# ARISE-Initiative/robosuite

Hardware: NVIDIA H100
Metric: env-steps/sec (device-timed) Panda-Lift OSC_POSE @4096 envs per GPU (higher is better)
Workload: dtype f32

## Files before the change

robosuite_b200/csrc/b2s_capi.cu:

```cuda
#include "../../include/b2s.h"
#include "b2s_unit.cuh"
#include "b2s_snapshot.cuh"

#include <cmath>
#include <cstdio>
#include <cstdlib>
#include <cstring>
#include <map>
#include <algorithm>
#include <string>
#include <type_traits>
#include <vector>

static thread_local std::string g_err;
static int fail(int code, const std::string& msg) { g_err = msg; return code; }
#define CUDA_TRY(x) do { cudaError_t e_ = (x); if (e_ != cudaSuccess) return fail(B2S_ERR_CUDA, std::string(#x) + ": " + cudaGetErrorString(e_)); } while (0)

struct BlobRec { char name[48]; int32_t dtype, ndim, shape[4]; int64_t off, nbytes; };
struct Blob {
  const char* p; size_t n;
  const BlobRec* find(const char* name) const {
    int64_t cnt; memcpy(&cnt, p + 8, 8);
    const BlobRec* r = (const BlobRec*)(p + 16);
    for (int64_t i = 0; i < cnt; i++) if (!strcmp(r[i].name, name)) return r + i;
    return nullptr;
  }
  bool has(const char* name) const { return find(name) != nullptr; }
  uint64_t hash() const;
  const double* f64(const char* name, int64_t* count = nullptr) const {
    const BlobRec* r = find(name);
    if (!r || r->dtype != 0) throw std::string("model blob: missing f64 field ") + name;
    if (count) *count = r->nbytes / 8;
    return (const double*)(p + r->off);
  }
  const int* i32(const char* name, int64_t* count = nullptr) const {
    const BlobRec* r = find(name);
    if (!r || r->dtype != 1) throw std::string("model blob: missing i32 field ") + name;
    if (count) *count = r->nbytes / 4;
    return (const int*)(p + r->off);
  }
  int scalar_i(const char* name) const { return i32(name)[0]; }
  double scalar_f(const char* name) const { return f64(name)[0]; }
};
static const uint64_t FNV_BASIS = 1469598103934665603ull;
static uint64_t fnv1a(uint64_t h, const void* p, size_t n) {
  const unsigned char* c = (const unsigned char*)p;
  for (size_t i = 0; i < n; i++) { h ^= c[i]; h *= 1099511628211ull; }
  return h;
}
uint64_t Blob::hash() const {
  int64_t cnt; memcpy(&cnt, p + 8, 8);
  const BlobRec* r = (const BlobRec*)(p + 16);
  uint64_t h = FNV_BASIS;
  for (int64_t i = 0; i < cnt; i++) {
    const char* nm = r[i].name;
    if (!strcmp(nm, "opt_maxcon") || !strcmp(nm, "opt_maxefc") || !strcmp(nm, "opt_maxcon_small") || !strcmp(nm, "opt_maxefc_small")) continue;
    h = fnv1a(h, nm, strnlen(nm, sizeof(r[i].name)) + 1);
    h = fnv1a(h, &r[i].dtype, sizeof(int32_t) * 6);
    h = fnv1a(h, p + r[i].off, (size_t)r[i].nbytes);
  }
  return h;
}

struct ArrayInfo { void* ptr; int dtype; int ndim; int64_t shape[4]; };
struct SnapSecHost { std::string name; int64_t off, count; int dtype; void* ptr; };
#define SNAP_MAXSEC 128

struct b2s_sim {
  int n_env = 0, device = 0, precision = B2S_F32;
  int num_sms = 1;
  cudaStream_t stream = 0;
  std::vector<void*> allocs;
  std::map<std::string, ArrayInfo> arrays;
  WSLayout lay[B2S_NLAY]{};
  int slot = -1;
  int mc_small = 0, me_small = 0;
  int osc_in_tail = 0;
  int wpb0 = 8, wpb5s = 8, wpb5l = 4;
  size_t smem0 = 0, smem5s = 0, smem5l = 0;
  DModel<float> mf{};
  DModel<double> md{};
  DState<float> sf{};
  DState<double> sd{};
  CtrlCfgDev ctrl{};
  int has_ctrl = 0;
  int wpb_fused = 4;
  size_t smem_fused = 0;
  int64_t launches = 0;
  int nq = 0, nv = 0, nu = 0, nbody = 0, ngeom = 0, nsite = 0, maxcon = 0, maxefc = 0, ncg = 0, hc_stride = 0;
  std::vector<double> qpos0;
  std::vector<int> site_bodyid, cgid;
  std::map<std::string, std::vector<std::string>> names;
  int has_obs = 0, export_env_step = 1, dirty = 1, mode = 0, ngroups = 8;
  int ctrl_split = 1;
  std::vector<cudaStream_t> gstreams;
  std::vector<cudaEvent_t> gevents;
  cudaEvent_t in_event = nullptr;
  void* action_buf = nullptr;
  std::map<long long, cudaGraphExec_t> graphs;
  PhaseIO pio[B2S_NPIO];
  std::map<std::string, Region> reg;
  int* uq_ring = nullptr; int* uq_ovf = nullptr; int* uq_ctr = nullptr; int uq_cap = 0;
  int uq_wpb = 0, uq_stride = 0, uq_stride_large = 0, uq_wpb_large = 0, uq_nlarge = 0, uq_grid = 0;
  size_t uq_smem = 0;
#ifdef B2S_INSTR
  unsigned long long* uq_prof = nullptr;
#endif
  std::vector<double> xpos0_h, xquat0_h;
  std::vector<int> body_weldid_h;
  std::vector<int> geom_type_h;
  std::vector<double> geom_size_h, geom_friction_h, geom_rbound_h, geom_aabb_h, body_mass_h, body_inertia_h, dof_iw_h, body_iw_h;
  std::vector<double> geom_solref_h, geom_solimp_h, dof_damping_h, dof_armature_h, dof_frictionloss_h;
  double meaninertia_h = 1;
  int sc_words = 0;
  PerturbEntry* pert_ent = nullptr;
  PerturbItem* pert_item = nullptr;
  int pert_nitems = 0;
  int layout_version = 0, snap_version = -1;
  std::vector<SnapSecHost> snap;
  size_t snap_row_bytes = 0;
  uint64_t snap_sig = 0, blob_hash = 0;
  SnapSec* snap_dev = nullptr;
  std::vector<int> obs_tab_h, task_tab_h;
};

template <typename F> static auto with_real(b2s_sim* s, F&& f) { return s->precision == B2S_F32 ? f(s->mf, s->sf) : f(s->md, s->sd); }
template <typename M> struct RealOf;
template <typename R> struct RealOf<DModel<R>> { using type = R; };
template <typename M> using real_of = typename RealOf<std::remove_cv_t<std::remove_reference_t<M>>>::type;
static size_t real_size(const b2s_sim* s) { return s->precision == B2S_F32 ? sizeof(float) : sizeof(double); }

static int launch_set_const(b2s_sim* s, const uint8_t* mask);

template <typename T> static T* dev_upload(b2s_sim* s, const std::vector<T>& h) {
  T* d = nullptr;
  size_t n = h.size() ? h.size() : 1;
  if (cudaMalloc(&d, n * sizeof(T)) != cudaSuccess) throw std::string("cudaMalloc failed");
  s->allocs.push_back(d);
  if (h.size()) cudaMemcpy(d, h.data(), h.size() * sizeof(T), cudaMemcpyHostToDevice);
  cudaStreamSynchronize(cudaStreamLegacy);
  return d;
}
template <typename R> static const R* up_f(b2s_sim* s, const Blob& b, const char* name) {
  int64_t n; const double* p = b.f64(name, &n);
  std::vector<R> h(n);
  for (int64_t i = 0; i < n; i++) h[i] = (R)p[i];
  return dev_upload(s, h);
}
static const int* up_i(b2s_sim* s, const Blob& b, const char* name) {
  int64_t n; const int* p = b.i32(name, &n);
  std::vector<int> h(p, p + n);
  return dev_upload(s, h);
}
template <typename R> static const R* up_vec(b2s_sim* s, const std::vector<double>& v) {
  std::vector<R> h(v.size());
  for (size_t i = 0; i < v.size(); i++) h[i] = (R)v[i];
  return dev_upload(s, h);
}

static void h_quat2mat(double* M, const double* q) {
  double w = q[0], x = q[1], y = q[2], z = q[3];
  M[0] = w * w + x * x - y * y - z * z; M[1] = 2 * (x * y - w * z); M[2] = 2 * (x * z + w * y);
// ... 325 lines not shown
  if (osc_in_tail && sc < 672) sc = 672;
  L.scratch_size = sc; L.scratch = B.take(sc);
  L.hdr = B.take(8);
  L.total = B.o;
}

static void layout_row(const Dims& d, WSLayout& L) {
  LayB B;
  int nv = d.nv, nb = d.nb, ncg = d.ncg, ns = d.ns;
  L = WSLayout{};
  L.xpos = B.take(3 * nb); L.xquat = B.take(4 * nb); L.cdof = B.take(6 * nv); L.cvel = B.take(6 * nb);
  L.M = B.take(nv * nv); L.bias = B.take(nv); L.passive = B.take(nv); L.spos = B.take(3 * ns); L.smat = B.take(9 * ns);
  L.gpos = B.take(3 * ncg); L.gmat = B.take(9 * ncg);
  L.hdr = B.take(8);
  L.total = B.o;
}

static void make_io(const Dims& d, const WSLayout& S, const WSLayout& ROW, std::initializer_list<const char*> names, Region* out, int& n, int* words) {
  int nv = d.nv, nb = d.nb, ncg = d.ncg, ns = d.ns;
  auto a4 = [](int x) { return (x + 3) & ~3; };
  std::vector<Region> v;
  for (const char* nm : names) {
    std::string k = nm;
    Region r{0, 0, 0, 0};
#define REG(name, field, len_) if (k == name) { r.off = S.field; r.goff = ROW.field; r.len = a4(len_); }
    REG("xpos", xpos, 3 * nb) REG("xquat", xquat, 4 * nb) REG("cdof", cdof, 6 * nv) REG("cvel", cvel, 6 * nb) REG("M", M, nv * nv)
    REG("bias", bias, nv) REG("passive", passive, nv) REG("spos", spos, 3 * ns) REG("smat", smat, 9 * ns)
    REG("gpos", gpos, 3 * ncg) REG("gmat", gmat, 9 * ncg)
#undef REG
    if (r.len > 0) v.push_back(r);
  }
  std::sort(v.begin(), v.end(), [](const Region& a, const Region& b) { return a.goff < b.goff; });
  n = 0;
  if (words) *words = 0;
  for (const Region& r : v) {
    if (n > 0 && out[n - 1].off + out[n - 1].len == r.off && out[n - 1].goff + out[n - 1].len == r.goff) out[n - 1].len += r.len;
    else { if (n >= B2S_MAXREG) throw std::string("too many workspace spans"); out[n++] = r; }
  }
  if (words) for (int k = 0; k < n; k++) *words += out[k].len;
}

static void build_layouts(b2s_sim* s, int ncg, int hc_stride) {
  Dims d{s->nq, s->nv, s->nu, s->nbody, ncg, s->nsite, hc_stride};
  layout_full(d, s->maxcon, s->maxefc, s->lay[LAY_FULL]);
  layout_p0(d, s->lay[LAY_P0]);
  layout_tail(d, s->mc_small, s->me_small, s->osc_in_tail != 0, s->lay[LAY_TS]);
  layout_tail(d, s->maxcon, s->maxefc, s->osc_in_tail != 0, s->lay[LAY_TL]);
  layout_row(d, s->lay[LAY_ROW]);
  for (int k = 0; k < B2S_NPIO; k++) s->pio[k] = PhaseIO{};
  const WSLayout& ROW = s->lay[LAY_ROW];
  make_io(d, s->lay[LAY_P0], ROW, {"xpos", "xquat", "cdof", "cvel", "M", "bias", "passive", "spos", "smat", "gpos", "gmat"},
          s->pio[PIO_P0].store, s->pio[PIO_P0].nstore, nullptr);
  for (int t = 0; t < 2; t++) {
    const WSLayout& T = s->lay[t ? LAY_TL : LAY_TS];
    PhaseIO& early = s->pio[t ? PIO_TL : PIO_TS];
    PhaseIO& late = s->pio[t ? PIO_TL_LATE : PIO_TS_LATE];
    if (s->osc_in_tail) make_io(d, T, ROW, {"cdof", "cvel", "M", "bias", "passive", "xpos", "xquat", "spos", "smat"}, early.load, early.nload, &early.load_words);
    else {
      make_io(d, T, ROW, {"cdof", "M", "bias", "passive"}, early.load, early.nload, &early.load_words);
      make_io(d, T, ROW, {"xpos", "xquat", "spos", "smat"}, late.load, late.nload, &late.load_words);
    }
  }
}

template <typename F> static cudaError_t optin_max_smem(F fn, int device, int* limit_out = nullptr) {
  cudaFuncAttributes a;
  cudaError_t e = cudaFuncGetAttributes(&a, fn);
  if (e != cudaSuccess) return e;
  int optin = 0;
  e = cudaDeviceGetAttribute(&optin, cudaDevAttrMaxSharedMemoryPerBlockOptin, device);
  if (e != cudaSuccess) return e;
  int lim = optin - (int)a.sharedSizeBytes;
  if (limit_out) *limit_out = lim;
  return cudaFuncSetAttribute(fn, cudaFuncAttributeMaxDynamicSharedMemorySize, lim);
}

static int fit_wpb(size_t per_warp, int cap) {
  int w = cap;
  while (w > 1 && per_warp * w > 226 * 1024) w--;
  return w;
}
static int choose_blocks(b2s_sim* s) {
  size_t rsz = real_size(s);
  size_t pw0 = s->lay[LAY_P0].total * rsz, pws = s->lay[LAY_TS].total * rsz, pwl = s->lay[LAY_TL].total * rsz, pwf = s->lay[LAY_FULL].fused_stride * rsz;
  if (std::max(std::max(pw0, pws), std::max(pwl, pwf)) > 226 * 1024) return fail(B2S_ERR_UNSUPPORTED, "model workspace exceeds shared memory");
  auto pick = [&](size_t pw, int lb_threads, int lb_blocks) {
    int cap = lb_threads / 32, w = cap;
    while (w > 1 && (pw * w + 1024) * lb_blocks > 228 * 1024) w--;
    if ((pw * w + 1024) * lb_blocks > 228 * 1024) w = fit_wpb(pw, cap);
    return w;
  };
  s->wpb0 = pick(pw0, P0_THREADS, P0_BLOCKS);
  s->wpb5s = pick(pws, TAIL_THREADS, TAIL_BLOCKS);
  s->wpb5l = fit_wpb(pwl, TAIL_THREADS / 32);
  s->smem0 = pw0 * s->wpb0; s->smem5s = pws * s->wpb5s; s->smem5l = pwl * s->wpb5l;
  int wf = fit_wpb(pwf, 16);
  s->wpb_fused = wf; s->smem_fused = pwf * wf;
  if (getenv("B2S_VERBOSE"))
    fprintf(stderr, "[b2s] slot %d words/warp: fused %d, P0 %d (%d warps/block), tail small %d [mc %d me %d] (%d warps/block), tail large %d [mc %d me %d] (%d), row %d\n",
            s->slot, s->lay[LAY_FULL].fused_stride, s->lay[LAY_P0].total, s->wpb0, s->lay[LAY_TS].total, s->mc_small, s->me_small, s->wpb5s,
            s->lay[LAY_TL].total, s->maxcon, s->maxefc, s->wpb5l, s->lay[LAY_ROW].total);
  return B2S_OK;
}

static b2s_sim* g_slots[64][B2S_NSLOT] = {{nullptr}};

static void keep_local_memory_pool() {
  unsigned flags = 0;
  if (cudaGetDeviceFlags(&flags) == cudaSuccess && (flags & cudaDeviceLmemResizeToMax)) return;
  const char* how = "unchanged";
  if (cudaSetDeviceFlags((flags & cudaDeviceMask) | cudaDeviceLmemResizeToMax) == cudaSuccess) how = "cudaSetDeviceFlags";
  else {
    cudaGetLastError();
    typedef int (*get_fn)(unsigned*);
    typedef int (*set_fn)(unsigned);
    void *fg = nullptr, *fs = nullptr;
    cudaDriverEntryPointQueryResult q1, q2;
    if (cudaGetDriverEntryPoint("cuCtxGetFlags", &fg, cudaEnableDefault, &q1) == cudaSuccess &&
        cudaGetDriverEntryPoint("cuCtxSetFlags", &fs, cudaEnableDefault, &q2) == cudaSuccess && fg && fs) {
      unsigned cf = 0;
      if (((get_fn)fg)(&cf) == 0 && ((set_fn)fs)(cf | 0x10u ) == 0) how = "cuCtxSetFlags";
    }
    cudaGetLastError();
  }
  if (getenv("B2S_VERBOSE")) fprintf(stderr, "[b2s] local-memory pool kept at high-water mark: %s\n", how);
}


extern "C" {

const char* b2s_last_error(void) { return g_err.c_str(); }

int b2s_create(const void* blob_host, size_t nbytes, int n_env, int device, int precision, b2s_sim** out) {
  if (!blob_host || !out || n_env <= 0) return fail(B2S_ERR_ARG, "b2s_create: bad argument");
  if (nbytes < 16 || memcmp(blob_host, "B2SMODEL", 8) != 0) return fail(B2S_ERR_MODEL, "b2s_create: not a model blob");
  if (precision != B2S_F32 && precision != B2S_F64) return fail(B2S_ERR_ARG, "b2s_create: precision must be B2S_F32 or B2S_F64");
  if (n_env >= (1 << 19)) return fail(B2S_ERR_UNSUPPORTED, "b2s_create: n_env must be below 524288 per handle (create several handles)");
  int ndev = 0;
  if (cudaGetDeviceCount(&ndev) != cudaSuccess || ndev == 0)
    return fail(B2S_ERR_CUDA, "b2s_create: no CUDA device available (this library has no CPU fallback)");
  CUDA_TRY(cudaSetDevice(device));
  keep_local_memory_pool();
  b2s_sim* s = new b2s_sim();
  s->n_env = n_env; s->device = device; s->precision = precision;
  if (cudaDeviceGetAttribute(&s->num_sms, cudaDevAttrMultiProcessorCount, device) != cudaSuccess) {
    b2s_destroy(s);
    return fail(B2S_ERR_CUDA, "b2s_create: cannot query the multiprocessor count");
  }
  Blob b{(const char*)blob_host, nbytes};
  try {
    s->nq = b.scalar_i("nq"); s->nv = b.scalar_i("nv"); s->nu = b.scalar_i("nu"); s->nbody = b.scalar_i("nbody");
    s->ngeom = b.scalar_i("ngeom"); s->nsite = b.scalar_i("nsite");
    s->blob_hash = b.hash();
    s->maxcon = b.has("opt_maxcon") ? b.scalar_i("opt_maxcon") : 32;
    s->maxefc = b.has("opt_maxefc") ? b.scalar_i("opt_maxefc") : 64;
    if (s->maxcon > 128) throw std::string("opt_maxcon > 128 not supported");
    const double* q0 = b.f64("qpos0");
    s->qpos0.assign(q0, q0 + s->nq);
    const int* sb = b.i32("site_bodyid");
    s->site_bodyid.assign(sb, sb + s->nsite);
    for (const char* ty : {"body", "joint", "geom", "site", "actuator", "mesh", "camera", "light"}) {
      std::string key = std::string("names_") + ty;
      if (!b.has(key.c_str())) continue;
      int64_t nc = 0; const int* cp = b.i32(key.c_str(), &nc);
      std::vector<std::string>& v = s->names[ty];
      std::string cur;
      for (int64_t i = 0; i < nc; i++) { if (cp[i] == '\n') { v.push_back(cur); cur.clear(); } else cur.push_back((char)cp[i]); }
      if (nc > 0) v.push_back(cur);
    }
    int nfl = 0;
    with_real(s, [&](auto& m, auto& st) {
      build_model(s, b, m);
      build_state(s, m, st);
      s->ncg = m.ncg; s->hc_stride = m.hc_stride; nfl = m.nfl;
    });
    s->mc_small = b.has("opt_maxcon_small") ? b.scalar_i("opt_maxcon_small") : s->maxcon;
    s->me_small = b.has("opt_maxefc_small") ? b.scalar_i("opt_maxefc_small") : s->maxefc;
    s->mc_small = std::min(std::max(s->mc_small, 4), s->maxcon);
    s->me_small = std::min(std::max(s->me_small, nfl + 8), s->maxefc);
    if (s->maxefc < nfl + 8) throw std::string("opt_maxefc too small for the model's friction-loss rows");
    for (int k = 0; k < B2S_NSLOT && s->slot < 0; k++)
      if (!g_slots[device & 63][k]) { g_slots[device & 63][k] = s; s->slot = k; }
    if (s->slot < 0) throw std::string("more than 8 live handles on one device");
    build_layouts(s, s->ncg, s->hc_stride);
  } catch (const std::string& e) {
    b2s_destroy(s);
    return fail(B2S_ERR_MODEL, "b2s_create: " + e);
  }
  if (choose_blocks(s) != B2S_OK) { b2s_destroy(s); return B2S_ERR_UNSUPPORTED; }
  {
    cudaError_t e1 = with_real(s, [&](auto& m, auto&) {
      using R = real_of<decltype(m)>;
      cudaError_t e = optin_max_smem(step_kernel<R>, device);
      if (e == cudaSuccess) e = optin_max_smem(phase0_kernel<R>, device);
      if (e == cudaSuccess) e = optin_max_smem(tail_kernel<R>, device);
      if (e == cudaSuccess) e = optin_max_smem(phase1_kernel<R>, device);
      return e;
    });
    if (e1 != cudaSuccess) { std::string msg = cudaGetErrorString(e1); b2s_destroy(s); return fail(B2S_ERR_CUDA, "cudaFuncSetAttribute: " + msg); }
  }
  *out = s;
  int rc = b2s_reset(s, nullptr);
  if (rc != 0) { b2s_destroy(s); *out = nullptr; return rc; }
  return B2S_OK;
}

void b2s_destroy(b2s_sim* s) {
  if (!s) return;
  if (s->slot >= 0 && g_slots[s->device & 63][s->slot] == s) g_slots[s->device & 63][s->slot] = nullptr;
  cudaSetDevice(s->device);
  cudaDeviceSynchronize();
  for (void* p : s->allocs) cudaFree(p);
  for (auto q : s->gstreams) cudaStreamDestroy(q);
  for (auto ev : s->gevents) cudaEventDestroy(ev);
  if (s->in_event) cudaEventDestroy(s->in_event);
  for (auto& kv : s->graphs) cudaGraphExecDestroy(kv.second);
  delete s;
}

int b2s_set_stream(b2s_sim* s, void* stream) {
  if (!s) return fail(B2S_ERR_ARG, "null handle");
  s->stream = (cudaStream_t)stream;
  return B2S_OK;
}

int b2s_set_export(b2s_sim* s, int flag) { if (!s) return fail(B2S_ERR_ARG, "null handle"); s->export_env_step = flag != 0; return B2S_OK; }

int64_t b2s_launch_count(const b2s_sim* s) { return s ? s->launches : 0; }

int b2s_array(b2s_sim* s, const char* name, void** dev_ptr, int* dtype, int* ndim, int64_t shape[4]) {
  if (!s || !name) return fail(B2S_ERR_ARG, "b2s_array: bad argument");
  auto it = s->arrays.find(name);
  if (it == s->arrays.end()) return fail(B2S_ERR_ARG, std::string("b2s_array: unknown array '") + name + "'");
  if (dev_ptr) *dev_ptr = it->second.ptr;
  if (dtype) *dtype = it->second.dtype;
  if (ndim) *ndim = it->second.ndim;
  if (shape) for (int k = 0; k < 4; k++) shape[k] = it->second.shape[k];
  return B2S_OK;
}

static int bind_constants(b2s_sim* s) {
  CUDA_TRY(cudaSetDevice(s->device));
  if (!s->dirty) return B2S_OK;
  const size_t k = (size_t)s->slot;
  int rc = with_real(s, [&](auto& m, auto& st) -> int {
    using D = DT<real_of<decltype(m)>>;
    CUDA_TRY(cudaMemcpyToSymbolAsync(D::model_bank(), &m, sizeof(m), k * sizeof(m), cudaMemcpyHostToDevice, s->stream));
    CUDA_TRY(cudaMemcpyToSymbolAsync(D::state_bank(), &st, sizeof(st), k * sizeof(st), cudaMemcpyHostToDevice, s->stream));
    return B2S_OK;
  });
  if (rc != B2S_OK) return rc;
  CUDA_TRY(cudaMemcpyToSymbolAsync(c_lay, s->lay, sizeof(s->lay), k * sizeof(s->lay), cudaMemcpyHostToDevice, s->stream));
  CUDA_TRY(cudaMemcpyToSymbolAsync(c_cc, &s->ctrl, sizeof(s->ctrl), k * sizeof(s->ctrl), cudaMemcpyHostToDevice, s->stream));
  CUDA_TRY(cudaMemcpyToSymbolAsync(c_pio, s->pio, sizeof(s->pio), k * sizeof(s->pio), cudaMemcpyHostToDevice, s->stream));
  s->dirty = 0;
  return B2S_OK;
}

static int rebuild_layouts(b2s_sim* s) {
  const bool osc = s->ctrl.kind == B2S_CTRL_OSC_POSE || s->ctrl.kind == B2S_CTRL_OSC_POSITION;
  int want = (osc && (!s->ctrl_split || s->mode == 2)) ? 1 : 0;
  if (want == s->osc_in_tail && s->smem0 != 0) return B2S_OK;
  s->uq_wpb = 0;
  s->osc_in_tail = want;
  try { build_layouts(s, s->ncg, s->hc_stride); } catch (const std::string& e) { return fail(B2S_ERR_MODEL, e); }
  int rc = choose_blocks(s);
  if (rc != B2S_OK) return rc;
  if (with_real(s, [](auto&, auto& st) { return st.wsg != nullptr; })) { cudaSetDevice(s->device); cudaDeviceSynchronize(); }
  for (auto& kv : s->graphs) cudaGraphExecDestroy(kv.second);
  s->graphs.clear();
  s->dirty = 1;
  return B2S_OK;
}

static int launch(b2s_sim* s, int phases, int nsub, const void* action = nullptr, const uint8_t* mask = nullptr) {
  int rc = bind_constants(s);
  if (rc != B2S_OK) return rc;
  int blocks = (s->n_env + s->wpb_fused - 1) / s->wpb_fused;
  with_real(s, [&](auto& m, auto&) {
    using R = real_of<decltype(m)>;
    step_kernel<R><<<blocks, s->wpb_fused * 32, s->smem_fused, s->stream>>>(phases, nsub, (const R*)action, s->slot, mask);
  });
  s->launches++;
  CUDA_TRY(cudaGetLastError());
  return B2S_OK;
}

}

template <typename R>
static int enqueue_group(b2s_sim* s, const DModel<R>& m, const DState<R>& st, int phases, int nsub, const R* action, int gi, int G, cudaStream_t q) {
  const int epaw = (EPA_AREA_WORDS(EPA_MAXV, EPA_MAXF) + m.stage_cap) * (int)sizeof(R);
  const int p1smem = std::max(epaw, (int)osc_smem_bytes<R>());
  const bool tiered = s->mc_small < s->maxcon || s->me_small < s->maxefc;
  int e0 = (int)((long long)s->n_env * gi / G), e1 = (int)((long long)s->n_env * (gi + 1) / G);
  Grp g{e0, e1 - e0, gi, 0, s->slot};
  int blocks0 = (g.nenv + s->wpb0 - 1) / s->wpb0, blocks5 = (g.nenv + s->wpb5s - 1) / s->wpb5s;
  int blocksL = std::min((g.nenv + s->wpb5l - 1) / s->wpb5l, 2 * s->num_sms);
  int nA = g.nenv * st.cl_maxa, nG = g.nenv * st.cl_maxg;
  const int cvx_blocks = std::max(s->num_sms, g.nenv / 2);
  const bool ctrl_ext = (phases & PH_CTRL_EXT) != 0;
  for (int sub = 0; sub < nsub; sub++) {
    g.sub = sub;
    CUDA_TRY(cudaMemsetAsync(st.cl_cnt + 8 * gi, 0, 8 * sizeof(int), q));
    phase0_kernel<R><<<blocks0, s->wpb0 * 32, s->smem0, q>>>(phases, g);
    P1Cfg c{std::min(nG, cvx_blocks), ctrl_ext ? (g.nenv + OSC_TPB - 1) / OSC_TPB : 0, sub};
    int nAb = (nA + 31) / 32;
    if (c.nG + c.nC + nAb > 0) phase1_kernel<R><<<c.nG + c.nC + nAb, 32, p1smem, q>>>(action, g, c);
    tail_kernel<R><<<blocks5, s->wpb5s * 32, s->smem5s, q>>>(phases, nsub, action, g, 0);
    if (tiered) tail_kernel<R><<<blocksL, s->wpb5l * 32, s->smem5l, q>>>(phases, nsub, action, g, 1);
  }
  CUDA_TRY(cudaGetLastError());
  return B2S_OK;
}

template <typename R> static int ensure_ws(b2s_sim* s, const DModel<R>& m, DState<R>& st) {
  if (!st.wsg) {
    R* p = nullptr;
    if (cudaMalloc(&p, (size_t)s->n_env * s->lay[LAY_ROW].total * sizeof(R)) != cudaSuccess) return fail(B2S_ERR_CUDA, "cudaMalloc(pipeline workspace) failed");
    cudaMemsetAsync(p, 0, (size_t)s->n_env * s->lay[LAY_ROW].total * sizeof(R), s->stream);
    s->allocs.push_back(p);
    st.wsg = p;
    size_t ne = (size_t)s->n_env;
    st.cl_cnt = dev_zeros<int>(s, 8 * 64);
    st.ovf_list = dev_zeros<int>(s, ne);
    st.cl_maxa = s->maxcon <= 32 ? 8 : (s->maxcon <= 48 ? 16 : CL_MAXA);
    st.cl_maxg = s->maxcon <= 32 ? 16 : CL_MAXG;
    st.cl_listA = dev_zeros<int>(s, ne * st.cl_maxa); st.cl_listG = dev_zeros<int>(s, ne * st.cl_maxg);
    st.cl_outA = dev_zeros<R>(s, ne * st.cl_maxa * CL_RECA); st.cl_outG = dev_zeros<R>(s, ne * st.cl_maxg * 8);
    st.cl_env = dev_zeros<int>(s, ne * CL_ENVW(st));
    st.gjk_cache = getenv("B2S_NO_GJK_CACHE") ? nullptr : dev_zeros<R>(s, ne * (size_t)m.npair * 3);
    s->action_buf = dev_zeros<R>(s, ne * 16);
#ifdef B2S_INSTR
    st.st_begin = dev_zeros<unsigned long long>(s, 64 * 32 * 8); st.st_end = dev_zeros<unsigned long long>(s, 64 * 32 * 8);
    st.stats = dev_zeros<int>(s, 512); st.cyc = dev_zeros<float>(s, ne * 64);
    s->arrays["st_begin"] = ArrayInfo{st.st_begin, B2S_I64, 1, {64 * 32 * 8, 0, 0, 0}};
    s->arrays["st_end"] = ArrayInfo{st.st_end, B2S_I64, 1, {64 * 32 * 8, 0, 0, 0}};
    s->arrays["stats"] = ArrayInfo{st.stats, B2S_I32, 1, {512, 0, 0, 0}};
    s->arrays["cyc"] = ArrayInfo{st.cyc, B2S_F32, 3, {(int64_t)ne, 32, 2, 0}};
    st.slowlog = dev_zeros<int>(s, 64 * 12);
    s->arrays["slowlog"] = ArrayInfo{st.slowlog, B2S_I32, 2, {64, 12, 0, 0}};
    s->uq_prof = dev_zeros<unsigned long long>(s, 16);
    s->arrays["unit_prof"] = ArrayInfo{s->uq_prof, B2S_I64, 1, {16, 0, 0, 0}};
#endif
    s->dirty = 1;
    s->layout_version++;
  }
  return B2S_OK;
}

static int launch_pipeline(b2s_sim* s, int phases, int nsub, const void* action) {
  return with_real(s, [&](auto& m, auto& st) -> int {
    using R = real_of<decltype(m)>;
    { int rc0 = ensure_ws(s, m, st); if (rc0 != B2S_OK) return rc0; }
#ifdef B2S_INSTR
    cudaMemsetAsync(st.st_begin, 0xff, sizeof(unsigned long long) * 64 * 32 * 8, s->stream);
    cudaMemsetAsync(st.st_end, 0, sizeof(unsigned long long) * 64 * 32 * 8, s->stream);
#endif
    const bool osc = s->ctrl.kind == B2S_CTRL_OSC_POSE || s->ctrl.kind == B2S_CTRL_OSC_POSITION;
    if ((phases & PH_CTRL) && osc && s->ctrl_split) phases |= PH_CTRL_EXT;
    { int rc2 = rebuild_layouts(s); if (rc2 != B2S_OK) return rc2; }
    int rc = bind_constants(s);
    if (rc != B2S_OK) return rc;
    const int G = std::min(s->ngroups, s->n_env);
    while ((int)s->gstreams.size() < G) {
      cudaStream_t st2; cudaEvent_t ev;
      CUDA_TRY(cudaStreamCreateWithFlags(&st2, cudaStreamNonBlocking));
      CUDA_TRY(cudaEventCreateWithFlags(&ev, cudaEventDisableTiming));
      s->gstreams.push_back(st2); s->gevents.push_back(ev);
    }
    if (!s->in_event) CUDA_TRY(cudaEventCreateWithFlags(&s->in_event, cudaEventDisableTiming));
    const bool tiered = s->mc_small < s->maxcon || s->me_small < s->maxefc;
    const int launches_per_call = G * nsub * (3 + (tiered ? 1 : 0));
    const R* act_in = (const R*)action;
    if (action) {
      int ad = s->ctrl.action_dim > 0 ? s->ctrl.action_dim : 1;
      if (ad > 16) return fail(B2S_ERR_UNSUPPORTED, "action_dim > 16");
      CUDA_TRY(cudaMemcpyAsync(s->action_buf, action, (size_t)s->n_env * ad * sizeof(R), cudaMemcpyDeviceToDevice, s->stream));
      act_in = (const R*)s->action_buf;
    }
    CUDA_TRY(cudaEventRecord(s->in_event, s->stream));
    for (int gi = 0; gi < G; gi++) {
      long long key = ((long long)phases << 28) | ((long long)(gi + 1) << 20) | (long long)nsub << 4 | (action ? 1 : 0);
      cudaStream_t q = s->gstreams[gi];
      auto it = s->graphs.find(key);
      if (it == s->graphs.end()) {
        cudaGraph_t graph = nullptr;
        cudaGraphExec_t exec = nullptr;
        CUDA_TRY(cudaStreamBeginCapture(q, cudaStreamCaptureModeRelaxed));
        rc = enqueue_group(s, m, st, phases, nsub, act_in, gi, G, q);
        cudaError_t ce = cudaStreamEndCapture(q, &graph);
        if (rc != B2S_OK) { if (graph) cudaGraphDestroy(graph); return rc; }
        if (ce != cudaSuccess) return fail(B2S_ERR_CUDA, std::string("cudaStreamEndCapture: ") + cudaGetErrorString(ce));
        CUDA_TRY(cudaGraphInstantiate(&exec, graph, 0));
        cudaGraphDestroy(graph);
        it = s->graphs.emplace(key, exec).first;
      }
      CUDA_TRY(cudaStreamWaitEvent(q, s->in_event, 0));
      CUDA_TRY(cudaGraphLaunch(it->second, q));
      CUDA_TRY(cudaEventRecord(s->gevents[gi], q));
      CUDA_TRY(cudaStreamWaitEvent(s->stream, s->gevents[gi], 0));
    }
    s->launches += launches_per_call;
    return B2S_OK;
  });
}

static int launch_unit(b2s_sim* s, int phases, int nsub, const void* action) {
  return with_real(s, [&](auto& m, auto& st) -> int {
    using R = real_of<decltype(m)>;
    { int rc0 = ensure_ws(s, m, st); if (rc0 != B2S_OK) return rc0; }
    { int rc2 = rebuild_layouts(s); if (rc2 != B2S_OK) return rc2; }
    const int total = s->n_env * nsub;
    if ((long long)s->n_env * nsub > (1ll << 30)) return fail(B2S_ERR_UNSUPPORTED, "unit-queue mode: n_env * nsub too large");
    if (total > s->uq_cap) {
      cudaStreamSynchronize(s->stream);
      int* p = nullptr;
      if (cudaMalloc(&p, sizeof(int) * (2 * (size_t)total + 8)) != cudaSuccess) return fail(B2S_ERR_CUDA, "cudaMalloc(unit ring) failed");
      s->allocs.push_back(p);
      s->uq_ring = p; s->uq_ovf = p + total; s->uq_ctr = p + 2 * (size_t)total; s->uq_cap = total;
#ifdef B2S_INSTR
      s->arrays["unit_ctr"] = ArrayInfo{s->uq_ctr, B2S_I32, 1, {8, 0, 0, 0}};
#endif
    }
    if (s->uq_wpb == 0) {
      const size_t rsz = sizeof(R);
      const bool tiered = s->mc_small < s->maxcon || s->me_small < s->maxefc;
      int stride = std::max(std::max(s->lay[LAY_P0].total, s->lay[LAY_TS].total), EPA_AREA_WORDS(EPA_MAXV, EPA_MAXF) + 24 + 384);
      stride = (stride + 3) & ~3;
      int stride_l = (s->lay[LAY_TL].total + 3) & ~3;
      CUDA_TRY(optin_max_smem(unit_kernel<R>, s->device));
      int best_w = 0, best_b = 0, best = 0;
      for (int w = UNIT_THREADS / 32; w >= 1; w--) {
        size_t sm = std::max((size_t)w * stride, tiered ? (size_t)stride_l : 0) * rsz;
        if (sm > 226 * 1024) continue;
        int b = 0;
        if (cudaOccupancyMaxActiveBlocksPerMultiprocessor(&b, unit_kernel<R>, w * 32, sm) != cudaSuccess) { cudaGetLastError(); continue; }
        if (w * b > best) { best = w * b; best_w = w; best_b = b; }
      }
      if (best == 0) return fail(B2S_ERR_UNSUPPORTED, "unit-queue mode: workspace does not fit shared memory");
      s->uq_stride = stride; s->uq_stride_large = stride_l;
      s->uq_smem = std::max((size_t)best_w * stride, tiered ? (size_t)stride_l : 0) * rsz;
      s->uq_wpb_large = tiered ? std::min(best_w, (int)(s->uq_smem / rsz / stride_l)) : 0;
      int slots = best_b * s->num_sms;
      int nl = tiered ? std::max(1, std::min(slots / 64, 12)) : 0;
      s->uq_nlarge = nl;
      if (best_w > s->n_env) best_w = s->n_env;
      s->uq_wpb = best_w;
      int small_blocks = std::min(std::max(slots - nl, 1), (s->n_env + best_w - 1) / best_w);
      s->uq_grid = nl + small_blocks;
      if (getenv("B2S_VERBOSE"))
        fprintf(stderr, "[b2s] unit-queue: %d warps/block x %d blocks/SM, %d words/warp (large role: %d words, %d warps/block, %d blocks), grid %d, smem %zu B\n",
                best_w, best_b, stride, stride_l, s->uq_wpb_large, nl, s->uq_grid, s->uq_smem);
    }
    int rc = bind_constants(s);
    if (rc != B2S_OK) return rc;
// ... 680 lines not shown
```

robosuite_b200/csrc/b2s_pipeline.cuh:

```cuda
#pragma once
#include "b2s_kernel.cuh"

DEV unsigned smem_u32(const void* p) { return (unsigned)__cvta_generic_to_shared(p); }
DEV void mbar_init(unsigned long long* bar) {
  asm volatile("mbarrier.init.shared::cta.b64 [%0], 1;" ::"r"(smem_u32(bar)));
  asm volatile("fence.mbarrier_init.release.cluster;" ::: "memory");
}
DEV void mbar_expect_tx(unsigned long long* bar, unsigned bytes) {
  asm volatile("mbarrier.arrive.expect_tx.shared::cta.b64 _, [%0], %1;" ::"r"(smem_u32(bar)), "r"(bytes) : "memory");
}
DEV void mbar_wait(unsigned long long* bar, unsigned parity) {
  asm volatile(
      "{\n"
      ".reg .pred p;\n"
      "WAIT_%=:\n"
      "mbarrier.try_wait.parity.shared::cta.b64 p, [%0], %1;\n"
      "@p bra DONE_%=;\n"
      "bra WAIT_%=;\n"
      "DONE_%=:\n"
      "}\n" ::"r"(smem_u32(bar)), "r"(parity) : "memory");
}
DEV void tma_load_1d(void* smem_dst, const void* gsrc, unsigned bytes, unsigned long long* bar) {
  asm volatile("cp.async.bulk.shared::cluster.global.mbarrier::complete_tx::bytes [%0], [%1], %2, [%3];" ::"r"(smem_u32(smem_dst)),
               "l"(gsrc), "r"(bytes), "r"(smem_u32(bar))
// ... 210 lines not shown
    if (worklist) s.cl_listA[baseA + i] = (env << 12) | cand[i];
    tab[2 + 2 * i] = cand[i]; tab[3 + 2 * i] = baseA + i;
  }
  for (int i = lane; i < ng; i += 32) {
    if (worklist) s.cl_listG[baseG + i] = (env << 12) | cand_g[i];
    tab[2 + 2 * (s.cl_maxa + i)] = cand_g[i]; tab[3 + 2 * (s.cl_maxa + i)] = baseG + i;
  }
  R* row = s.wsg + E * RL.total;
  if (lane == 0) reinterpret_cast<int*>(row + RL.hdr)[2] = warn;
  __syncwarp();
  ws_store(e, row, c_pio[e.slot][PIO_P0]);
}

#define TAIL_NCON(pk) ((pk) & 255)
#define TAIL_WARN(pk) (((pk) >> 8) & 255)
#define TAIL_NEFC(pk) (((pk) >> 16) & 0x3fff)
#define TAIL_OVF(pk) ((pk) >> 30)
template <typename R> DEV int tail_rows(Eng<R>& e, int env, unsigned long long* bar, unsigned& parity) {
  const DModel<R>& m = e.model();
  const DState<R>& s = e.state();
  const WSLayout& L = e.lay();
  const WSLayout& RL = c_lay[e.slot][LAY_ROW];
  const int lane = e.lane;
  const bool tiered = L.mc < m.maxcon || L.me < m.maxefc;
  const size_t E = env;
  e.env = env;
  const R* row = s.wsg + E * RL.total;
  const int warn = reinterpret_cast<const int*>(row + RL.hdr)[2];
  ws_load(e, row, c_pio[e.slot][e.lid == LAY_TL ? PIO_TL : PIO_TS], bar, parity);
  load_row(e.p(L.qpos), s.qpos + E * m.nq, m.nq, lane);
  load_row(e.p(L.qvel), s.qvel + E * m.nv, m.nv, lane);
  load_row(e.p(L.ctrl), s.ctrl + E * m.nu, m.nu, lane);
  load_row(e.p(L.qacc_ws), s.qacc_ws + E * m.nv, m.nv, lane);
  __syncwarp();
  int wl = 0;
  const int ncon = gather_contacts(e, env, wl);
  const int nefc = (tiered && (wl & 4)) ? 0 : make_constraint(e, ncon, wl);
  wl = warp_or_i(wl);
  const int ovf = (tiered && (wl & 12)) ? 1 : 0;
  return (ncon & 255) | (((warn | wl) & 255) << 8) | ((nefc & 0x3fff) << 16) | (ovf << 30);
}

template <typename R> DEV void tail_ctrl(Eng<R>& e, int env, int sub, const R* action) {
  const DModel<R>& m = e.model();
  const DState<R>& s = e.state();
  const WSLayout& L = e.lay();
  const size_t E = env;
  CtrlState<R> cs;
  ctrl_load(e, cs, env);
  ctrl_run(e, cs, env, sub == 0 ? action : (const R*)nullptr);
  for (int i = e.lane; i < m.nu; i += 32) s.ctrl[E * m.nu + i] = e.p(L.ctrl)[i];
  if (sub == 0) ctrl_store(e, cs, env);
  __syncwarp();
}

template <typename R> DEV int tail_accel(Eng<R>& e) {
  e.actuation((R*)nullptr);
  return e.acceleration() ? 1 : 0;
}
template <typename R> DEV int tail_newton(Eng<R>& e, int nefc, int ncon) {
  int warn = 0;
  solve(e, nefc, ncon, warn);
  return warn;
}

template <typename R>
DEV void tail_finish(Eng<R>& e, int env, int sub, int nsub, int phases, int ncon, int warn, unsigned long long* bar, unsigned& parity) {
  const DState<R>& s = e.state();
  e.env = env;
  R time = s.time[env];
  if (!(phases & PH_NOINTEGRATE)) {
    { int eb = e.euler(&time); if (eb & 32) warn |= 32; else if (eb) warn |= 2; }
  }
  if ((phases & PH_OBS) && e.ccfg().obs_dim > 0 && sub == nsub - 1) {
    ws_load(e, s.wsg + (size_t)env * c_lay[e.slot][LAY_ROW].total, c_pio[e.slot][e.lid == LAY_TL ? PIO_TL_LATE : PIO_TS_LATE], bar, parity);
    write_obs(e, env, (phases & PH_NOINTEGRATE) != 0);
    write_task(e, env, ncon);
  }
  store_state(e, env, time, warn);
}

constexpr int P0_THREADS = 256, P0_BLOCKS = 2;
constexpr int TAIL_THREADS = 256, TAIL_BLOCKS = 2;

template <typename R>
__global__ void __launch_bounds__(P0_THREADS, P0_BLOCKS) phase0_kernel(int phases, Grp g) {
  const DState<R>& s = cstate<R>(g.slot);
  const WSLayout& L = c_lay[g.slot][LAY_P0];
  extern __shared__ __align__(16) unsigned char smem_raw[];
  R* smem = reinterpret_cast<R*>(smem_raw);
  int warp = threadIdx.x >> 5, lane = threadIdx.x & 31, wpb = blockDim.x >> 5;
  int env = blockIdx.x * wpb + warp;
  INSTR_BEGIN(s, g, 0)
#ifdef B2S_INSTR
  long long instr_t0 = clock64();
#endif
  if (env >= g.nenv) return;
  env += g.env0;
  Eng<R> e(smem + (size_t)warp * L.total, lane, g.slot, LAY_P0);
  int na, ng;
  const int warn = phase0_env(e, env, na, ng);
  int baseA = 0, baseG = 0;
  if (lane == 0) {
    if (na) baseA = g.env0 * s.cl_maxa + atomicAdd(CLC(s, g), na);
    if (ng) baseG = g.env0 * s.cl_maxg + atomicAdd(CLC(s, g) + 1, ng);
  }
  baseA = __shfl_sync(B2S_FULL, baseA, 0);
  baseG = __shfl_sync(B2S_FULL, baseG, 0);
  phase0_publish(e, env, na, ng, warn, baseA, baseG, true);
#ifdef B2S_INSTR
  if (lane == 0 && s.cyc) s.cyc[((size_t)env * 32 + (g.sub & 31)) * 2] = (float)(clock64() - instr_t0);
#endif
  INSTR_END(s, g, 0)
}

template <typename R>
__global__ void __launch_bounds__(TAIL_THREADS, TAIL_BLOCKS) tail_kernel(int phases, int nsub, const R* action, Grp g, int tier) {
  const DState<R>& s = cstate<R>(g.slot);
  const int lid = tier ? LAY_TL : LAY_TS;
  const WSLayout& L = c_lay[g.slot][lid];
  extern __shared__ __align__(16) unsigned char smem_raw[];
  R* smem = reinterpret_cast<R*>(smem_raw);
  const int warp = threadIdx.x >> 5, lane = threadIdx.x & 31, wpb = blockDim.x >> 5, sub = g.sub;
  INSTR_BEGIN(s, g, tier ? 5 : 3)
  __shared__ unsigned long long mbar[32];
  if (lane == 0) mbar_init(&mbar[warp]);
  __syncwarp();
  unsigned parity = 0;
  Eng<R> e(smem + (size_t)warp * L.total, lane, g.slot, lid);
  int* clc = CLC(s, g);
  for (int iter = 0;; iter++) {
    int env;
    if (tier == 0) {
      if (iter > 0) break;
      env = blockIdx.x * wpb + warp;
      if (env >= g.nenv) break;
      env += g.env0;
    } else {
      int item = 0;
      if (lane == 0) item = atomicAdd(clc + 4, 1);
      item = __shfl_sync(B2S_FULL, item, 0);
      if (item >= clc[2]) break;
      env = s.ovf_list[g.env0 + item];
    }
#ifdef B2S_INSTR
    long long instr_t0 = clock64();
#endif
    const int pk = tail_rows(e, env, &mbar[warp], parity);
    if (TAIL_OVF(pk)) {
      if (lane == 0) s.ovf_list[g.env0 + atomicAdd(clc + 2, 1)] = env;
      __syncwarp();
      continue;
    }
    const int ncon = TAIL_NCON(pk), nefc = TAIL_NEFC(pk);
    int warn = TAIL_WARN(pk);
    if ((phases & PH_CTRL) && !(phases & PH_CTRL_EXT)) tail_ctrl(e, env, sub, action);
    warn |= tail_accel(e);
    warn |= tail_newton(e, nefc, ncon);
    tail_finish(e, env, sub, nsub, phases, ncon, warn, &mbar[warp], parity);
#ifdef B2S_INSTR
    if (lane == 0 && s.cyc) s.cyc[((size_t)env * 32 + (sub & 31)) * 2 + 1] = (float)(clock64() - instr_t0);
    if (lane == 0 && s.stats) { atomicAdd(s.stats + 32 + min(ncon, 128), 1); atomicAdd(s.stats + 176 + min(nefc, 320), 1); if (tier) atomicAdd(s.stats + 19, 1); }
#endif
  }
  INSTR_END(s, g, tier ? 5 : 3)
}
```

robosuite_b200/csrc/b2s_types.cuh:

```cuda
#pragma once
#include <cuda_runtime.h>
#include <stdint.h>

#define B2S_FULL 0xffffffffu
#define B2S_MOV 8

enum { JNT_FREE = 0, JNT_BALL = 1, JNT_SLIDE = 2, JNT_HINGE = 3 };
enum { G_PLANE = 0, G_HFIELD, G_SPHERE, G_CAPSULE, G_ELLIPSOID, G_CYLINDER, G_BOX, G_MESH };
enum { C_FRICTION = 1, C_LIMIT = 3, C_FRICTIONLESS = 5, C_ELLIPTIC = 7 };
enum { DK_FREE_T = 0, DK_FREE_R = 1, DK_SLIDE = 2, DK_HINGE = 3 };

enum {
  PH_STEP1 = 1,
  PH_STEP2 = 2,
  PH_NOINTEGRATE = 4,
  PH_EXPORT = 8,
  PH_CTRL = 16,
  PH_CTRL_EXT = 512,
  PH_OBS = 64
};

template <typename R>
struct DModel {
  int nq, nv, nu, nbody, njnt, ngeom, nsite, npair, ncg, nment, maxdepth, maxcon, maxefc, nmocap, nfl, nlim, hc_stride, max_treesize;
  int stage_cap;
  R timestep, impratio, density, viscosity, tolerance, meaninertia;
  int iterations, ls_iterations;
  R gravity[3];
  const int *body_parentid, *body_jntid, *body_dofnum, *body_dofadr, *body_weldid, *body_subtree_end, *body_depth;
  const R *body_pos, *body_quat, *body_ipos, *body_iquat, *body_mass, *body_inertia, *body_invweight0;
  const R *body_xpos0, *body_xquat0;
  const int *jnt_type, *jnt_qposadr, *jnt_dofadr, *jnt_bodyid, *jnt_limited;
  const R *jnt_pos, *jnt_axis, *jnt_range, *jnt_solref, *jnt_solimp, *qpos0;
  const int *dof_bodyid, *dof_jntid, *dof_parentid, *dof_kind, *dof_cddstart, *fl_dof, *lim_jnt, *dof_treebase, *dof_treesize, *body_treeid;
  const unsigned long long* body_dofmask;
  const R *dof_armature, *dof_damping, *dof_frictionloss, *dof_solref, *dof_solimp, *dof_invweight0;
  const int *ment_i, *ment_j;
  const int *geom_type, *geom_bodyid, *geom_condim, *geom_dataid, *geom_priority, *geom_cgid, *cg_geom;
  const R *geom_size, *geom_pos, *geom_quat, *geom_friction, *geom_solmix, *geom_solref, *geom_solimp, *geom_rbound,
      *geom_aabb;
  const int* pair_geom;
  const int *mesh_vertadr, *mesh_vertnum;
  const R* mesh_vert;
  const int* site_bodyid;
  const R *site_pos, *site_quat;
  const int *act_trnid, *act_ctrllimited, *act_forcelimited, *act_biastype;
  const R *act_ctrlrange, *act_forcerange, *act_gear, *act_gainprm, *act_biasprm;
};

template <typename R>
struct DState {
  int n_env;
  R *qpos, *qvel, *qacc, *qacc_ws, *ctrl, *time;
  R *xpos, *xquat, *xmat, *site_xpos, *site_xmat, *geom_xpos, *geom_xmat, *qM, *qfrc_bias, *qfrc_passive,
      *qfrc_actuator, *qfrc_constraint, *qfrc_smooth, *qacc_smooth, *actuator_force, *cdof;
  int *ncon, *contact_geom, *contact_dim, *nefc, *efc_type, *warn, *solver_niter;
  R *contact_dist, *contact_pos, *contact_frame, *contact_friction, *contact_solref, *contact_solimp, *efc_J, *efc_force,
      *efc_aref, *efc_D, *efc_R;
  R *goal_pos, *goal_ori, *init_qpos_arm, *grip_state;
  R* ctrl_torque;
  R* jv_state;
  R* obs;
  R* wsg;
  int* cl_cnt;
  int* ovf_list;
  int cl_maxa, cl_maxg;
  int* cl_listA;
  int* cl_listG;
  R* cl_outA;
  R* cl_outG;
  R* gjk_cache;
  int* cl_env;
  int* obs_fresh;
  int n_ov, ov_body[4];
  R* ov_pos[4];
  R* ov_quat[4];
  int n_mg, n_mb;
  short mg_id[B2S_MOV], mb_id[B2S_MOV];
  R *mg_size, *mg_fric, *mg_rbound, *mg_aabb;
  R *mb_mass, *mb_inertia;
  R *mg_solref, *mg_solimp;
  R *dof_iw, *body_iw, *mean_inertia;
  R *dof_damp, *dof_arm, *dof_floss;
  R* task_vec;
  R* task_out;
  unsigned long long* st_begin;
  unsigned long long* st_end;
  int* stats;
  float* cyc;
  int* slowlog;
};

struct WSLayout {
  int qpos, qvel, qacc, qacc_ws, ctrl;
  int xpos, xquat, xmat, xipos;
  int cdof, cdofdot, cinert, cvel, frne, ffl;
  int M, H;
  int bias, passive, qact, qsmooth, qaccs, qcon;
  int gpos, gmat, spos, smat;
  int c_pos, c_frame, c_dist, c_fric, c_solref, c_solimp, c_mu, c_int;
  int J, e_D, e_R, e_aref, e_jar, e_jv, e_force, e_floss, e_int;
  int Ma, grad, search, Mv;
  int scratch, scratch_size;
  int fused_stride;
  int hdr;
  int total;
  int mc, me;
};

#define B2S_NSLOT 8
enum { LAY_FULL = 0, LAY_P0 = 1, LAY_TS = 2, LAY_TL = 3, LAY_ROW = 4, B2S_NLAY = 5 };

struct Region { int off, goff, len, dyn; };
enum { PIO_P0 = 0, PIO_TS = 1, PIO_TS_LATE = 2, PIO_TL = 3, PIO_TL_LATE = 4, B2S_NPIO = 5 };
#define CL_MAXA 64
#define CL_MAXG 32
#define CL_RECA 58
#define CL_ENVW(s) (2 + 2 * ((s).cl_maxa + (s).cl_maxg))
#define B2S_MAXREG 12
struct PhaseIO { int nload, nstore, load_words, load_dyn; Region load[B2S_MAXREG], store[B2S_MAXREG]; };

enum { OB_QPOS = 0, OB_COS_QPOS, OB_SIN_QPOS, OB_QVEL, OB_QACC, OB_SITE_POS, OB_BODY_POS, OB_BODY_QUAT_XYZW, OB_SITE_QUAT_XYZW,
       OB_BODY_MINUS_SITE, OB_SITE_MINUS_SITE, OB_BODY_QUAT_REL_SITE_XYZW, OB_ZERO, OB_BODY_MINUS_BODY,
       OB_REL_POS_LAG, OB_REL_QUAT_LAG };

struct CtrlCfgDev {
  int kind, action_dim, n_arm, eef_site, base_site, n_grip, uncouple;
  int obs_dim; const int* obs_op; const int* obs_a; const int* obs_b;
  int task_body, task_site; unsigned long long mask_left, mask_right, mask_obj;
  int task_body2; unsigned long long mask_obj2;
  int n_objs; unsigned long long mask_objs[4];
  int task_dim; const int* task_op; const int* task_a; const int* task_b;
  double jv_kp[8], jv_ki[8], jv_kd[8], jv_in_max[8], jv_in_min[8], jv_out_max[8], jv_out_min[8], jv_vel_lo, jv_vel_hi;
  int jv_use_vel_limits, jv_torque_comp;
  int arm_dof[8], arm_qpos[8], arm_act[8], grip_act[4];
  double grip_sign[4], grip_speed, kp[6], kd[6], input_max[6], input_min[6], output_max[6], output_min[6], null_kp;
};

__constant__ DModel<float> c_model_f[B2S_NSLOT];
__constant__ DModel<double> c_model_d[B2S_NSLOT];
__constant__ DState<float> c_state_f[B2S_NSLOT];
__constant__ DState<double> c_state_d[B2S_NSLOT];
__constant__ WSLayout c_lay[B2S_NSLOT][B2S_NLAY];
__constant__ CtrlCfgDev c_cc[B2S_NSLOT];
__constant__ PhaseIO c_pio[B2S_NSLOT][B2S_NPIO];
template <typename R> __device__ __forceinline__ const DModel<R>& cmodel(int slot);
template <> __device__ __forceinline__ const DModel<float>& cmodel<float>(int slot) { return c_model_f[slot]; }
template <> __device__ __forceinline__ const DModel<double>& cmodel<double>(int slot) { return c_model_d[slot]; }
// ... 4 lines not shown
```

Baseline: 301,400.

## Handle tail overflow envs in-block instead of separate large-tier launch

Merges the two-tier tail kernel into one launch. Each block first runs the small-workspace path for its warps, then reuses the same shared memory with the large layout to redo the environments that overflowed. This removes the second kernel launch, the global overflow list and its atomics, and it moves the counter memset out of the substep loop. It also adds an optional 512-thread wide tail variant when the workspace fits, at the cost of a block barrier and serialized overflow handling by fewer warps.

```diff
diff --git a/robosuite_b200/csrc/b2s_capi.cu b/robosuite_b200/csrc/b2s_capi.cu
--- a/robosuite_b200/csrc/b2s_capi.cu
+++ b/robosuite_b200/csrc/b2s_capi.cu
@@ -76,8 +76,8 @@
   int slot = -1;
   int mc_small = 0, me_small = 0;
   int osc_in_tail = 0;
-  int wpb0 = 8, wpb5s = 8, wpb5l = 4;
-  size_t smem0 = 0, smem5s = 0, smem5l = 0;
+  int wpb0 = 8, wpb5 = 8, stride5 = 0, stride5l = 0, nlw5 = 1, tail_wide = 0;
+  size_t smem0 = 0, smem5 = 0;
   DModel<float> mf{};
   DModel<double> md{};
   DState<float> sf{};
@@ -569,7 +569,10 @@
 }
 static int choose_blocks(b2s_sim* s) {
   size_t rsz = real_size(s);
-  size_t pw0 = s->lay[LAY_P0].total * rsz, pws = s->lay[LAY_TS].total * rsz, pwl = s->lay[LAY_TL].total * rsz, pwf = s->lay[LAY_FULL].fused_stride * rsz;
+  auto a4 = [](int x) { return (x + 3) & ~3; };
+  s->stride5 = a4(s->lay[LAY_TS].total);
+  s->stride5l = a4(s->lay[LAY_TL].total);
+  size_t pw0 = s->lay[LAY_P0].total * rsz, pws = s->stride5 * rsz, pwl = s->stride5l * rsz, pwf = s->lay[LAY_FULL].fused_stride * rsz;
   if (std::max(std::max(pw0, pws), std::max(pwl, pwf)) > 226 * 1024) return fail(B2S_ERR_UNSUPPORTED, "model workspace exceeds shared memory");
   auto pick = [&](size_t pw, int lb_threads, int lb_blocks) {
     int cap = lb_threads / 32, w = cap;
@@ -578,15 +581,19 @@
     return w;
   };
   s->wpb0 = pick(pw0, P0_THREADS, P0_BLOCKS);
-  s->wpb5s = pick(pws, TAIL_THREADS, TAIL_BLOCKS);
-  s->wpb5l = fit_wpb(pwl, TAIL_THREADS / 32);
-  s->smem0 = pw0 * s->wpb0; s->smem5s = pws * s->wpb5s; s->smem5l = pwl * s->wpb5l;
+  s->wpb5 = pick(pws, TAIL_THREADS, TAIL_BLOCKS);
+  const int wide_w = TAIL_WIDE_THREADS / 32;
+  s->tail_wide = pws * wide_w <= 160 * 1024;
+  if (s->tail_wide) s->wpb5 = wide_w;
+  s->smem5 = std::max(pws * s->wpb5, pwl);
+  s->nlw5 = std::max(1, std::min(s->wpb5, (int)(s->smem5 / pwl)));
+  s->smem0 = pw0 * s->wpb0;
   int wf = fit_wpb(pwf, 16);
   s->wpb_fused = wf; s->smem_fused = pwf * wf;
   if (getenv("B2S_VERBOSE"))
-    fprintf(stderr, "[b2s] slot %d words/warp: fused %d, P0 %d (%d warps/block), tail small %d [mc %d me %d] (%d warps/block), tail large %d [mc %d me %d] (%d), row %d\n",
-            s->slot, s->lay[LAY_FULL].fused_stride, s->lay[LAY_P0].total, s->wpb0, s->lay[LAY_TS].total, s->mc_small, s->me_small, s->wpb5s,
-            s->lay[LAY_TL].total, s->maxcon, s->maxefc, s->wpb5l, s->lay[LAY_ROW].total);
+    fprintf(stderr, "[b2s] slot %d words/warp: fused %d, P0 %d (%d warps/block), tail small %d [mc %d me %d] (%d warps/block, wide %d), tail large %d [mc %d me %d] (%d), row %d\n",
+            s->slot, s->lay[LAY_FULL].fused_stride, s->lay[LAY_P0].total, s->wpb0, s->lay[LAY_TS].total, s->mc_small, s->me_small, s->wpb5, s->tail_wide,
+            s->lay[LAY_TL].total, s->maxcon, s->maxefc, s->nlw5, s->lay[LAY_ROW].total);
   return B2S_OK;
 }
 
@@ -680,7 +687,8 @@
       using R = real_of<decltype(m)>;
       cudaError_t e = optin_max_smem(step_kernel<R>, device);
       if (e == cudaSuccess) e = optin_max_smem(phase0_kernel<R>, device);
-      if (e == cudaSuccess) e = optin_max_smem(tail_kernel<R>, device);
+      if (e == cudaSuccess) e = optin_max_smem(tail_kernel<R, TAIL_THREADS>, device);
+      if (e == cudaSuccess) e = optin_max_smem(tail_kernel<R, TAIL_WIDE_THREADS>, device);
       if (e == cudaSuccess) e = optin_max_smem(phase1_kernel<R>, device);
       return e;
     });
@@ -779,23 +787,21 @@
 static int enqueue_group(b2s_sim* s, const DModel<R>& m, const DState<R>& st, int phases, int nsub, const R* action, int gi, int G, cudaStream_t q) {
   const int epaw = (EPA_AREA_WORDS(EPA_MAXV, EPA_MAXF) + m.stage_cap) * (int)sizeof(R);
   const int p1smem = std::max(epaw, (int)osc_smem_bytes<R>());
-  const bool tiered = s->mc_small < s->maxcon || s->me_small < s->maxefc;
   int e0 = (int)((long long)s->n_env * gi / G), e1 = (int)((long long)s->n_env * (gi + 1) / G);
   Grp g{e0, e1 - e0, gi, 0, s->slot};
-  int blocks0 = (g.nenv + s->wpb0 - 1) / s->wpb0, blocks5 = (g.nenv + s->wpb5s - 1) / s->wpb5s;
-  int blocksL = std::min((g.nenv + s->wpb5l - 1) / s->wpb5l, 2 * s->num_sms);
+  int blocks0 = (g.nenv + s->wpb0 - 1) / s->wpb0, blocks5 = (g.nenv + s->wpb5 - 1) / s->wpb5;
   int nA = g.nenv * st.cl_maxa, nG = g.nenv * st.cl_maxg;
   const int cvx_blocks = std::max(s->num_sms, g.nenv / 2);
   const bool ctrl_ext = (phases & PH_CTRL_EXT) != 0;
+  CUDA_TRY(cudaMemsetAsync(st.cl_cnt + 8 * gi, 0, 8 * sizeof(int), q));
   for (int sub = 0; sub < nsub; sub++) {
     g.sub = sub;
-    CUDA_TRY(cudaMemsetAsync(st.cl_cnt + 8 * gi, 0, 8 * sizeof(int), q));
     phase0_kernel<R><<<blocks0, s->wpb0 * 32, s->smem0, q>>>(phases, g);
     P1Cfg c{std::min(nG, cvx_blocks), ctrl_ext ? (g.nenv + OSC_TPB - 1) / OSC_TPB : 0, sub};
     int nAb = (nA + 31) / 32;
     if (c.nG + c.nC + nAb > 0) phase1_kernel<R><<<c.nG + c.nC + nAb, 32, p1smem, q>>>(action, g, c);
-    tail_kernel<R><<<blocks5, s->wpb5s * 32, s->smem5s, q>>>(phases, nsub, action, g, 0);
-    if (tiered) tail_kernel<R><<<blocksL, s->wpb5l * 32, s->smem5l, q>>>(phases, nsub, action, g, 1);
+    if (s->tail_wide) tail_kernel<R, TAIL_WIDE_THREADS><<<blocks5, s->wpb5 * 32, s->smem5, q>>>(phases, nsub, action, g, s->stride5, s->stride5l, s->nlw5);
+    else tail_kernel<R, TAIL_THREADS><<<blocks5, s->wpb5 * 32, s->smem5, q>>>(phases, nsub, action, g, s->stride5, s->stride5l, s->nlw5);
   }
   CUDA_TRY(cudaGetLastError());
   return B2S_OK;
@@ -810,7 +816,6 @@
     st.wsg = p;
     size_t ne = (size_t)s->n_env;
     st.cl_cnt = dev_zeros<int>(s, 8 * 64);
-    st.ovf_list = dev_zeros<int>(s, ne);
     st.cl_maxa = s->maxcon <= 32 ? 8 : (s->maxcon <= 48 ? 16 : CL_MAXA);
     st.cl_maxg = s->maxcon <= 32 ? 16 : CL_MAXG;
     st.cl_listA = dev_zeros<int>(s, ne * st.cl_maxa); st.cl_listG = dev_zeros<int>(s, ne * st.cl_maxg);
@@ -857,8 +862,7 @@
       s->gstreams.push_back(st2); s->gevents.push_back(ev);
     }
     if (!s->in_event) CUDA_TRY(cudaEventCreateWithFlags(&s->in_event, cudaEventDisableTiming));
-    const bool tiered = s->mc_small < s->maxcon || s->me_small < s->maxefc;
-    const int launches_per_call = G * nsub * (3 + (tiered ? 1 : 0));
+    const int launches_per_call = G * nsub * 3;
     const R* act_in = (const R*)action;
     if (action) {
       int ad = s->ctrl.action_dim > 0 ? s->ctrl.action_dim : 1;
diff --git a/robosuite_b200/csrc/b2s_pipeline.cuh b/robosuite_b200/csrc/b2s_pipeline.cuh
--- a/robosuite_b200/csrc/b2s_pipeline.cuh
+++ b/robosuite_b200/csrc/b2s_pipeline.cuh
@@ -316,6 +316,7 @@
 
 constexpr int P0_THREADS = 256, P0_BLOCKS = 2;
 constexpr int TAIL_THREADS = 256, TAIL_BLOCKS = 2;
+constexpr int TAIL_WIDE_THREADS = 512;
 
 template <typename R>
 __global__ void __launch_bounds__(P0_THREADS, P0_BLOCKS) phase0_kernel(int phases, Grp g) {
@@ -349,53 +350,49 @@
 }
 
 template <typename R>
-__global__ void __launch_bounds__(TAIL_THREADS, TAIL_BLOCKS) tail_kernel(int phases, int nsub, const R* action, Grp g, int tier) {
-  const DState<R>& s = cstate<R>(g.slot);
-  const int lid = tier ? LAY_TL : LAY_TS;
-  const WSLayout& L = c_lay[g.slot][lid];
+DEVN int tail_env(R* area, int lane, int lid, Grp g, int env, int nsub, int phases, const R* action, unsigned long long* bar, unsigned& parity) {
+  const int sub = g.sub;
+  Eng<R> e(area, lane, g.slot, lid);
+#ifdef B2S_INSTR
+  const DState<R>& s = cstate<R>(g.slot);
+  long long instr_t0 = clock64();
+#endif
+  const int pk = tail_rows(e, env, bar, parity);
+  if (TAIL_OVF(pk)) return 1;
+  const int ncon = TAIL_NCON(pk), nefc = TAIL_NEFC(pk);
+  int warn = TAIL_WARN(pk);
+  if ((phases & PH_CTRL) && !(phases & PH_CTRL_EXT)) tail_ctrl(e, env, sub, action);
+  warn |= tail_accel(e);
+  warn |= tail_newton(e, nefc, ncon);
+  tail_finish(e, env, sub, nsub, phases, ncon, warn, bar, parity);
+#ifdef B2S_INSTR
+  if (lane == 0 && s.cyc) s.cyc[((size_t)env * 32 + (sub & 31)) * 2 + 1] = (float)(clock64() - instr_t0);
+  if (lane == 0 && s.stats) { atomicAdd(s.stats + 32 + min(ncon, 128), 1); atomicAdd(s.stats + 176 + min(nefc, 320), 1); if (lid == LAY_TL) atomicAdd(s.stats + 19, 1); }
+#endif
+  return 0;
+}
+
+template <typename R, int THREADS>
+__global__ void __launch_bounds__(THREADS, THREADS == TAIL_WIDE_THREADS ? 1 : TAIL_BLOCKS) tail_kernel(int phases, int nsub, const R* action, Grp g, int stride, int stride_l, int nlw) {
+  const DState<R>& s = cstate<R>(g.slot);
   extern __shared__ __align__(16) unsigned char smem_raw[];
   R* smem = reinterpret_cast<R*>(smem_raw);
-  const int warp = threadIdx.x >> 5, lane = threadIdx.x & 31, wpb = blockDim.x >> 5, sub = g.sub;
-  INSTR_BEGIN(s, g, tier ? 5 : 3)
+  const int warp = threadIdx.x >> 5, lane = threadIdx.x & 31, wpb = blockDim.x >> 5;
+  INSTR_BEGIN(s, g, 3)
   __shared__ unsigned long long mbar[32];
+  __shared__ int ovf[32];
+  if (blockIdx.x == 0 && threadIdx.x == 0) { int* c = CLC(s, g); c[0] = 0; c[1] = 0; c[3] = 0; }
   if (lane == 0) mbar_init(&mbar[warp]);
   __syncwarp();
   unsigned parity = 0;
-  Eng<R> e(smem + (size_t)warp * L.total, lane, g.slot, lid);
-  int* clc = CLC(s, g);
-  for (int iter = 0;; iter++) {
-    int env;
-    if (tier == 0) {
-      if (iter > 0) break;
-      env = blockIdx.x * wpb + warp;
-      if (env >= g.nenv) break;
-      env += g.env0;
-    } else {
-      int item = 0;
-      if (lane == 0) item = atomicAdd(clc + 4, 1);
-      item = __shfl_sync(B2S_FULL, item, 0);
-      if (item >= clc[2]) break;
-      env = s.ovf_list[g.env0 + item];
-    }
-#ifdef B2S_INSTR
-    long long instr_t0 = clock64();
-#endif
-    const int pk = tail_rows(e, env, &mbar[warp], parity);
-    if (TAIL_OVF(pk)) {
-      if (lane == 0) s.ovf_list[g.env0 + atomicAdd(clc + 2, 1)] = env;
-      __syncwarp();
-      continue;
-    }
-    const int ncon = TAIL_NCON(pk), nefc = TAIL_NEFC(pk);
-    int warn = TAIL_WARN(pk);
-    if ((phases & PH_CTRL) && !(phases & PH_CTRL_EXT)) tail_ctrl(e, env, sub, action);
-    warn |= tail_accel(e);
-    warn |= tail_newton(e, nefc, ncon);
-    tail_finish(e, env, sub, nsub, phases, ncon, warn, &mbar[warp], parity);
-#ifdef B2S_INSTR
-    if (lane == 0 && s.cyc) s.cyc[((size_t)env * 32 + (sub & 31)) * 2 + 1] = (float)(clock64() - instr_t0);
-    if (lane == 0 && s.stats) { atomicAdd(s.stats + 32 + min(ncon, 128), 1); atomicAdd(s.stats + 176 + min(nefc, 320), 1); if (tier) atomicAdd(s.stats + 19, 1); }
-#endif
-  }
-  INSTR_END(s, g, tier ? 5 : 3)
-}
+  const int env = g.env0 + blockIdx.x * wpb + warp;
+  int o = -1;
+  if (env < g.env0 + g.nenv && tail_env<R>(smem + (size_t)warp * stride, lane, LAY_TS, g, env, nsub, phases, action, &mbar[warp], parity)) o = env;
+  if (lane == 0) ovf[warp] = o;
+  asm volatile("fence.proxy.async.shared::cta;" ::: "memory");
+  __syncthreads();
+  if (warp < nlw)
+    for (int k = warp; k < wpb; k += nlw)
+      if (ovf[k] >= 0) tail_env<R>(smem + (size_t)warp * stride_l, lane, LAY_TL, g, ovf[k], nsub, phases, action, &mbar[warp], parity);
+  INSTR_END(s, g, 3)
+}
diff --git a/robosuite_b200/csrc/b2s_types.cuh b/robosuite_b200/csrc/b2s_types.cuh
--- a/robosuite_b200/csrc/b2s_types.cuh
+++ b/robosuite_b200/csrc/b2s_types.cuh
@@ -63,7 +63,6 @@
   R* obs;
   R* wsg;
   int* cl_cnt;
-  int* ovf_list;
   int cl_maxa, cl_maxg;
   int* cl_listA;
   int* cl_listG;
```

Result: faster. 322,800 (median of 6 runs) (+7.1%).
